# qianlim/CAPE

Measured on NVIDIA H100. Metric: meshes/sec fwd+bwd CAPE-affineconv nz64, higher is better.
Workload: dtype f32

## Files before the change

cape_b200/csrc/ellconv_dw_tc.cu:

```cuda
#include "common.cuh"
#include "ellconv_params.cuh"
#include "tc_common.cuh"

namespace cape {

namespace {

using namespace tc;

constexpr int DW_THREADS = 256;
constexpr int DW_KCH = 32;
constexpr int DW_A_TILE = 128 * 128;

struct DwTcParams {
  int rows_out, ncols, F, src_rows, src_stride;
  long long total_rows, rows_per_split;
  const float* src;
  OpView op;
  const float* g;
  float* out;
  long long out_rs;
  int nsplit, accumulate;
};

template <int BN>
struct DwCfg {
  static constexpr int G_TILE = BN * 128;
  static constexpr int STAGE = 2 * DW_A_TILE + 2 * G_TILE;
  static constexpr int SMEM_BYTES = 1024 + 2 * STAGE;
};

template <int BN>
__global__ void __launch_bounds__(DW_THREADS, BN <= 64 ? 2 : 1) dw_wg_kernel(const __grid_constant__ DwTcParams p) {
  using Cfg = DwCfg<BN>;
  constexpr int NA = BN / 2;
  constexpr int GQ = BN / 32;
  extern __shared__ uint8_t smem_raw[];
  char* smem = reinterpret_cast<char*>((reinterpret_cast<uintptr_t>(smem_raw) + 1023) & ~(uintptr_t)1023);

  const int tid = threadIdx.x, warp = tid >> 5, lane = tid & 31, wgi = tid >> 7, wt = tid & 127;
  const int ftile = blockIdx.x * 128;
  const int col0 = blockIdx.z * BN;
  const long long rbeg = (long long)blockIdx.y * p.rows_per_split;
  const long long rend = min(p.total_rows, rbeg + p.rows_per_split);
  const long long nchunks = (rend - rbeg + DW_KCH - 1) / DW_KCH;

  float4 ra[4], rg[GQ];
  auto load_chunk = [&](long long kc) {
    const long long R = rbeg + kc * DW_KCH + lane;
    const bool live = R < rend;
    const long long Q = live ? R : rbeg;
    const int n = (int)(Q / p.rows_out), r = (int)(Q % p.rows_out);
    const float* base = p.src + (size_t)n * p.src_rows * p.src_stride;
#pragma unroll
    for (int i = 0; i < 4; ++i) {
      const int f = ftile + 4 * (warp + 8 * i);
      float4 v = make_float4(0.f, 0.f, 0.f, 0.f);
      if (live && f < p.F) {
        if (p.op.idx == nullptr) v = ldg4(base + (size_t)r * p.src_stride + f);
        else ell_gather4(p.op, r, base + f, (size_t)p.src_stride, v);
      }
      ra[i] = v;
    }
#pragma unroll
    for (int i = 0; i < GQ; ++i) {
      const int c = col0 + 4 * (warp + 8 * i);
      rg[i] = make_float4(0.f, 0.f, 0.f, 0.f);
      if (live && c < p.ncols) rg[i] = ldg4(p.g + (size_t)R * p.ncols + c);
    }
  };
  auto store_chunk = [&](int stage) {
    char* a_hi = smem + (size_t)stage * Cfg::STAGE;
    char* a_lo = a_hi + DW_A_TILE;
    char* g_hi = a_lo + DW_A_TILE;
    char* g_lo = g_hi + Cfg::G_TILE;
#pragma unroll
    for (int i = 0; i < 4; ++i) {
      const int m = 4 * (warp + 8 * i);
      split_store1(ra[i].x, a_hi, a_lo, sw_off(m, lane));
      split_store1(ra[i].y, a_hi, a_lo, sw_off(m + 1, lane));
      split_store1(ra[i].z, a_hi, a_lo, sw_off(m + 2, lane));
      split_store1(ra[i].w, a_hi, a_lo, sw_off(m + 3, lane));
    }
#pragma unroll
    for (int i = 0; i < GQ; ++i) {
      const int m = 4 * (warp + 8 * i);
      split_store1(rg[i].x, g_hi, g_lo, sw_off(m, lane));
      split_store1(rg[i].y, g_hi, g_lo, sw_off(m + 1, lane));
      split_store1(rg[i].z, g_hi, g_lo, sw_off(m + 2, lane));
      split_store1(rg[i].w, g_hi, g_lo, sw_off(m + 3, lane));
    }
  };

  float acc[NA];
#pragma unroll
  for (int i = 0; i < NA; ++i) acc[i] = 0.f;

  if (nchunks > 0) {
    load_chunk(0);
    store_chunk(0);
    fence_proxy_async();
    __syncthreads();
    for (long long kc = 0;; ++kc) {
      const int stage = (int)(kc & 1);
      const uint32_t base = smem_u32(smem + (size_t)stage * Cfg::STAGE);
      const uint32_t a_hi = base + (uint32_t)(wgi * 64 * 128), a_lo = a_hi + DW_A_TILE;
      const uint32_t g_hi = base + 2 * DW_A_TILE, g_lo = g_hi + Cfg::G_TILE;
      wgmma_fence();
      fence_acc(acc);
      mma3_chunk<BN>(acc, a_hi, a_lo, g_hi, g_lo, 1);
      wgmma_commit();
      const bool more = kc + 1 < nchunks;
      if (more) {
        load_chunk(kc + 1);
        store_chunk(stage ^ 1);
      }
      wgmma_wait_all();
      fence_acc(acc);
      if (!more) break;
      fence_proxy_async();
      __syncthreads();
    }
  }

  float* out = p.out + (p.nsplit > 1 ? (size_t)blockIdx.y * p.F * p.out_rs : 0);
  const bool vec2 = (p.out_rs % 2 == 0) && ((reinterpret_cast<uintptr_t>(out) & 7u) == 0);
#pragma unroll
  for (int i = 0; i < NA; i += 2) {
    const int f = ftile + wgi * 64 + frag_row(wt, i);
    const int c = col0 + frag_col(wt, i);
    if (f >= p.F || c >= p.ncols) continue;
    float* o = out + (size_t)f * p.out_rs + c;
    if (p.nsplit == 1 && p.accumulate) {
      o[0] += acc[i];
      o[1] += acc[i + 1];
    } else if (vec2) {
      *reinterpret_cast<float2*>(o) = make_float2(acc[i], acc[i + 1]);
    } else {
      o[0] = acc[i];
      o[1] = acc[i + 1];
    }
  }
}

template <int BN>
int launch_dw(const DwTcParams& p, int ftiles, cudaStream_t st) {
  using Cfg = DwCfg<BN>;
  static bool configured = false;
  if (!configured) {
    CAPE_CHECK_CUDA(cudaFuncSetAttribute(dw_wg_kernel<BN>, cudaFuncAttributeMaxDynamicSharedMemorySize, Cfg::SMEM_BYTES));
    configured = true;
  }
  dim3 grid(ftiles, p.nsplit, (p.ncols + BN - 1) / BN);
  dw_wg_kernel<BN><<<grid, DW_THREADS, Cfg::SMEM_BYTES, st>>>(p);
  CAPE_CHECK_CUDA(cudaGetLastError());
  count_launches(1);
  return 1;
}

}

int launch_ellconv_dw_tc(const cape_topology* t, const cape_dw_args* a, const OpView& op, int* nsplit_out,
                         cudaStream_t st) {
  if (!tensor_cores_enabled()) return 0;
  if (a->ncols % 32 != 0 || a->ncols < 32 || a->ncols > 512) return 0;
  if (a->F % 4 != 0 || a->F < 32 || a->src_stride % 4 != 0 || !aligned16(a->src) || !aligned16(a->g)) return 0;
  DwTcParams p{};
  p.rows_out = a->rows_out; p.ncols = a->ncols; p.F = a->F; p.src_rows = a->src_rows; p.src_stride = a->src_stride;
  p.total_rows = (long long)a->N * a->rows_out;
  if (p.total_rows < 4096 || p.total_rows >= (1LL << 31)) return 0;
  p.src = a->src; p.op = op; p.g = a->g;
  const int BN = a->ncols <= 32 ? 32 : (a->ncols <= 64 ? 64 : (a->ncols <= 128 ? 128 : 256));
  const int ftiles = (a->F + 127) / 128, ctiles = (a->ncols + BN - 1) / BN;
  long long nsplit = (2LL * t->sm_count + ftiles * ctiles - 1) / (ftiles * ctiles);
  const long long max_by_rows = (p.total_rows + 511) / 512;
  if (nsplit > max_by_rows) nsplit = max_by_rows;
  const long long per = (long long)a->F * a->ncols * (long long)sizeof(float);
  if (nsplit > 1 && nsplit * per > t->workspace_bytes) nsplit = t->workspace_bytes / per;
  if (nsplit < 1) nsplit = 1;
  long long rps = (p.total_rows + nsplit - 1) / nsplit;
  rps = (rps + DW_KCH - 1) / DW_KCH * DW_KCH;
  nsplit = (p.total_rows + rps - 1) / rps;
  p.rows_per_split = rps; p.nsplit = (int)nsplit; p.accumulate = a->accumulate;
  if (nsplit == 1) { p.out = a->dw; p.out_rs = a->dw_stride; }
  else { p.out = (float*)t->workspace; p.out_rs = a->ncols; }
  *nsplit_out = (int)nsplit;
  if (BN == 32) return launch_dw<32>(p, ftiles, st);
  if (BN == 64) return launch_dw<64>(p, ftiles, st);
  if (BN == 128) return launch_dw<128>(p, ftiles, st);
  return launch_dw<256>(p, ftiles, st);
}

}
```

cape_b200/csrc/tc_common.cuh:

```cuda
#pragma once
#include <stdint.h>
#include "../../include/cape_b200.h"
#include "wgmma_tf32.cuh"

namespace cape {
namespace tc {

__device__ __forceinline__ uint32_t smem_u32(const void* p) { return (uint32_t)__cvta_generic_to_shared(p); }

__device__ __forceinline__ uint64_t make_desc(uint32_t smem_addr) {
  return (uint64_t)((smem_addr >> 4) & 0x3fffu) | (1ull << 16) | ((uint64_t)(1024 >> 4) << 32) | (1ull << 62);
}

__device__ __forceinline__ uint32_t sw_off(int m, int k) {
  return (uint32_t)(m * 128 + ((((k >> 2) ^ (m & 7)) << 4) | ((k & 3) << 2)));
}

__device__ __forceinline__ void fence_proxy_async() { asm volatile("fence.proxy.async.shared::cta;" ::: "memory"); }
__device__ __forceinline__ void wgmma_fence() { asm volatile("wgmma.fence.sync.aligned;" ::: "memory"); }
__device__ __forceinline__ void wgmma_commit() { asm volatile("wgmma.commit_group.sync.aligned;" ::: "memory"); }
__device__ __forceinline__ void wgmma_wait_all() { asm volatile("wgmma.wait_group.sync.aligned 0;" ::: "memory"); }

__device__ __forceinline__ void mbar_init(uint64_t* bar, int count) {
  asm volatile("mbarrier.init.shared::cta.b64 [%0], %1;" ::"r"(smem_u32(bar)), "r"(count) : "memory");
}
__device__ __forceinline__ void mbar_arrive(uint64_t* bar) {
  asm volatile("mbarrier.arrive.shared::cta.b64 _, [%0];" ::"r"(smem_u32(bar)) : "memory");
}
__device__ __forceinline__ void mbar_wait(uint64_t* bar, uint32_t parity) {
  uint32_t done;
  do {
    asm volatile("{\n\t.reg .pred p;\n\tmbarrier.try_wait.parity.shared::cta.b64 p, [%1], %2;\n\tselp.u32 %0, 1, 0, p;\n\t}"
                 : "=r"(done) : "r"(smem_u32(bar)), "r"(parity) : "memory");
  } while (!done);
}
__device__ __forceinline__ void named_bar_sync(int id, int nthreads) {
  asm volatile("bar.sync %0, %1;" ::"r"(id), "r"(nthreads) : "memory");
}
template <int N>
__device__ __forceinline__ void setmaxnreg_dec() { asm volatile("setmaxnreg.dec.sync.aligned.u32 %0;" ::"n"(N)); }
template <int N>
__device__ __forceinline__ void setmaxnreg_inc() { asm volatile("setmaxnreg.inc.sync.aligned.u32 %0;" ::"n"(N)); }

template <int N>
__device__ __forceinline__ void fence_acc(float (&d)[N]) {
#pragma unroll
  for (int i = 0; i < N; ++i) asm volatile("" : "+f"(d[i])::"memory");
}

__device__ __forceinline__ float tf32_hi(float x) { return __uint_as_float(__float_as_uint(x) & 0xffffe000u); }

__device__ __forceinline__ void split_store4(float4 v, char* hi_tile, char* lo_tile, uint32_t off) {
  float4 h, l;
  h.x = tf32_hi(v.x); l.x = v.x - h.x;
  h.y = tf32_hi(v.y); l.y = v.y - h.y;
  h.z = tf32_hi(v.z); l.z = v.z - h.z;
  h.w = tf32_hi(v.w); l.w = v.w - h.w;
  *reinterpret_cast<float4*>(hi_tile + off) = h;
  *reinterpret_cast<float4*>(lo_tile + off) = l;
}
__device__ __forceinline__ void split_store1(float v, char* hi_tile, char* lo_tile, uint32_t off) {
  const float h = tf32_hi(v);
  *reinterpret_cast<float*>(hi_tile + off) = h;
  *reinterpret_cast<float*>(lo_tile + off) = v - h;
}

template <int N>
__device__ __forceinline__ void mma3_chunk(float (&d)[N / 2], uint32_t a_hi, uint32_t a_lo, uint32_t b_hi,
                                           uint32_t b_lo, int scale_first) {
#pragma unroll
  for (int ks = 0; ks < 4; ++ks) {
    const uint32_t adv = 32u * ks;
    wg::mma_tf32<N>(d, make_desc(a_hi + adv), make_desc(b_hi + adv), ks == 0 ? scale_first : 1);
    wg::mma_tf32<N>(d, make_desc(a_lo + adv), make_desc(b_hi + adv), 1);
    wg::mma_tf32<N>(d, make_desc(a_hi + adv), make_desc(b_lo + adv), 1);
  }
}

__device__ __forceinline__ int frag_row(int t, int i) { return 16 * (t >> 5) + ((t & 31) >> 2) + 8 * ((i >> 1) & 1); }
__device__ __forceinline__ int frag_col(int t, int i) { return 8 * (i >> 2) + 2 * (t & 3) + (i & 1); }

}
}
```

cape_b200/network.py:

```python
import math
import os

import numpy as np
import torch

from . import _lib
from . import engine as E
from . import topology as topo
from .engine import (ACT_LEAKY, ACT_NONE, EPI_AFFINE, EPI_DUALMASK, EPI_LINEAR, EPI_SLOPE, ConvSite, Topology,
                     act_bwd, axpy, cheb_call, cheb_dw, colsum, gemm)
from .params import init_params, is_d_param, is_g_param, param_specs


ADAM_BETA1, ADAM_BETA2, ADAM_EPS = float(np.float32(0.9)), float(np.float32(0.999)), 1e-8


def _pad4(n):
    return (n + 3) // 4 * 4


class ParamStore:

    def __init__(self, specs, names, device):
        self.names = list(names)
        self.shapes = {n: tuple(specs[n]) for n in self.names}
        self.offsets = {}
        off = 0
        for n in self.names:
            self.offsets[n] = off
            off += _pad4(int(np.prod(self.shapes[n])))
        self.size = max(off, 4)
        self.flat = torch.zeros(self.size, device=device)
        self.grad = torch.zeros(self.size, device=device)
        self.mom = torch.zeros(self.size, device=device)
        self.lo = torch.zeros(self.size, device=device)
        self.var = None

    def add_adam_slot(self):
        if self.var is None:
            self.var = torch.zeros(self.size, device=self.flat.device)

    def lo_of(self, t):
        off = (t.data_ptr() - self.flat.data_ptr()) // 4
        if t.data_ptr() < self.flat.data_ptr() or off + t.numel() > self.size or not t.is_contiguous():
            return None
        return self.lo[off: off + t.numel()].view(t.shape)

    def _view(self, buf, n):
        k = int(np.prod(self.shapes[n]))
        return buf[self.offsets[n]: self.offsets[n] + k]

    def w(self, n):
        return self._view(self.flat, n)

    def g(self, n):
        return self._view(self.grad, n)

    def load(self, values):
        for n in self.names:
            self.w(n).copy_(torch.as_tensor(np.asarray(values[n], np.float32).reshape(-1)))

    def export(self, buf=None):
        buf = self.flat if buf is None else buf
        return {n: self._view(buf, n).detach().cpu().numpy().reshape(self.shapes[n]).copy() for n in self.names}


class Arena:

    def __init__(self):
        self.reqs = []
        self.buf = None

    def request(self, *shape):
        self.reqs.append(shape)
        return len(self.reqs) - 1

    def build(self, device):
        offs, off = [], 0
        for s in self.reqs:
            offs.append(off)
            off += _pad4(int(np.prod(s)))
        self.buf = torch.zeros(max(off, 4), device=device)
        self.views = [self.buf[o: o + int(np.prod(s))].view(*s) for o, s in zip(offs, self.reqs)]

    def get(self, i):
        return self.views[i]

    def zero(self):
        self.buf.zero_()


def choose_dw_mode(F, Fout, K, rows_in, rows_out, need_dx, stash=True):
    dense_ok = F % 4 == 0 and F >= 32 and Fout % 32 == 0 and Fout <= 512
    if not (dense_ok and stash):
        return "gather"
    if rows_out < rows_in:
        return "aside"
    if need_dx and (rows_in < rows_out or (K * Fout <= 512 and F >= Fout)):
        return "gside"
    return "aside"


def choose_forms(F, C, Fout, K, rows_in, rows_out, affine, need_dx, dw_mode, plain, name="", env=None):
    env = os.environ if env is None else env
    thin = F <= 4 or Fout <= 4
    split_ok = not thin and not plain and F % 16 == 0 and Fout % 16 == 0 and F >= 32 and Fout >= 32
    fwd_mode, dx_mode = "fused", "fused"
    basis_ok = C == 0 and not affine and dw_mode == "aside"
    if split_ok:
        if basis_ok and K >= 3 and rows_out < rows_in:
            fwd_mode = "basis"
        elif (C > 0 or affine) and rows_in < rows_out:
            fwd_mode = "contract"
        if (need_dx and not affine and dw_mode == "aside" and K * F <= 512
                and (Fout > F or (rows_out < rows_in and Fout == F and F >= 128))):
            dx_mode = "contract"
        if need_dx and dw_mode == "gside" and rows_in < rows_out and Fout >= 128:
            dx_mode = "basis"
    fm, dm = env.get("CAPE_FWD_MODE", ""), env.get("CAPE_DX_MODE", "")
    for item in filter(None, env.get("CAPE_MODES", "").split(",")):
        key, val = item.split("=")
        if key == name + ":fwd":
            fm = val
        elif key == name + ":dx":
            dm = val
    if fm and (fm == "fused" or (split_ok and (fm != "basis" or basis_ok))):
        fwd_mode = fm
    if dm and need_dx and (dm == "fused" or (split_ok and (dm != "basis" or dw_mode == "gside")
                                             and (dm != "contract" or (dw_mode != "gside" and not affine)))):
        dx_mode = dm
    return fwd_mode, dx_mode


class ChebLayer:

    def __init__(self, net, site, F, C, Fout, W, gW, bias=None, gbias=None, act=ACT_NONE, Wa=None, gWa=None,
                 bias_per_row=False, need_dx=True, maxN=1, n_cs_slots=1, name=""):
        self.net, self.tp, self.site, self.name = net, net.tp, site, name
        if (bias is not None or act != ACT_NONE) and not site.pool_is_selection:
            raise NotImplementedError("%s: the down-sampling matrix is not a pure row selection, so pooling cannot be "
                                      "folded in front of the bias/activation (lib/models.py:164-168 applies them "
                                      "before the pool)" % name)
        self.F, self.C, self.Fout, self.K = F, C, Fout, site.K
        K = self.K
        self.W3, self.gW3 = W.view(F + C, K, Fout), gW.view(F + C, K, Fout)
        self.W, self.bias, self.gbias, self.act = W, bias, gbias, act
        self.bias_per_row = bias_per_row
        self.affine = Wa is not None
        if self.affine:
            self.Wa, self.Wa2, self.gWa2 = Wa, Wa.view(F + C, Fout), gWa.view(F + C, Fout)
        self.need_dx = need_dx
        dev = W.device
        A = 1 if self.affine else 0
        self.Wt, self.Wt_lo = torch.empty(K + A, Fout, F, device=dev), torch.empty(K + A, Fout, F, device=dev)
        self.W3_lo = net.lo_of(W).view(F + C, K, Fout)
        net.wprep.add(W, F, K, Fout, wt=self.Wt[:K], wt_lo=self.Wt_lo[:K])
        if self.affine:
            self.Wa2_lo = net.lo_of(Wa).view(F + C, Fout)
            net.wprep.add(Wa, F, 1, Fout, wt=self.Wt[K:], wt_lo=self.Wt_lo[K:])
        self.dw_mode = choose_dw_mode(F, Fout, K, site.rows_in, site.rows_out, need_dx,
                                      os.environ.get("CAPE_DW_STASH", "1") != "0")
        self.stash_a, self.stash_g, self.stash_ga = [None] * K, [None] * K, None
        if self.dw_mode == "aside":
            nz = [k for k in range(K) if site.ops[k] != -1]
            self.stash_all = torch.empty(max(len(nz), 1), maxN, site.rows_out, F, device=dev)
            self.stash_a = [None] * K
            for j, k in enumerate(nz):
                self.stash_a[k] = self.stash_all[j]
        elif self.dw_mode == "gside":
            self.g_merged = K > 1 and K * Fout <= 512
            if self.g_merged:
                self.Hg = torch.empty(maxN, site.rows_in, K * Fout, device=dev)
                self.stash_g = [self.Hg[:, :, k * Fout:(k + 1) * Fout] for k in range(K)]
            else:
                self.stash_g = [None if site.opsT[k] == -1 else torch.empty(maxN, site.rows_in, Fout, device=dev)
                                for k in range(K)]
            if self.affine and site.opsT[0] != -1:
                self.stash_ga = torch.empty(maxN, site.rows_in, Fout, device=dev)
        self.fwd_mode, self.dx_mode = choose_forms(F, C, Fout, K, site.rows_in, site.rows_out, self.affine, need_dx,
                                                   self.dw_mode, all(o == -1 for o in site.ops), name)
        if self.dx_mode == "contract":
            self.Wk, self.Wk_lo = torch.empty(K, F, Fout, device=dev), torch.empty(K, F, Fout, device=dev)
            net.wprep.add(W, F, K, Fout, wk=self.Wk, wk_lo=self.Wk_lo)
            net.scratch_req(maxN * site.rows_out * K * F)
        if self.fwd_mode == "contract":
            net.scratch_req(maxN * site.rows_in * (K + A) * Fout)
        self.cs_ops = []
        if bias is not None and not bias_per_row:
            self.cs_ops.append(-1)
        self.cs_cond0 = len(self.cs_ops)
        if C:
            self.cs_ops += list(site.ops)
        self.cs_id = [net.arena.request(maxN, max(len(self.cs_ops), 1), Fout) for _ in range(n_cs_slots)]
        self.csa_id = net.arena.request(maxN, 1, Fout) if (self.affine and C) else None

    def alg_bytes(self, N, what):
        s, Fin, Fo, K = self.site, self.F + self.C, self.Fout, self.K
        wbytes = 4 * Fin * K * Fo + (12 * s.nnz if K > 1 else 0)
        conv = 4 * N * s.M * (Fin + Fo) + wbytes
        if self.affine:
            conv += 4 * N * s.M * (Fin + Fo) + 4 * Fin * Fo
            wbytes += 4 * Fin * Fo
        res = 0
        if s.ref_unpool:
            res += 4 * N * Fin * (s.ref_rows_in + s.M)
        if s.ref_pool:
            res += 4 * N * Fo * (s.M + s.ref_rows_out)
        if what in ("fwd", "dx"):
            return conv + res
        return 4 * N * s.M * Fin * (2 if self.affine else 1) + wbytes

    def _split(self):
        return E.tensor_cores_enabled(self.tp)

    def fwd(self, x, ycat, out, out2=None):
        N = x.shape[0]
        s, F, C, K, Fout = self.site, self.F, self.C, self.K, self.Fout
        assert x.shape[1] == s.rows_in and x.shape[2] >= F and out.shape[1] == s.rows_out
        sx = x.shape[2]
        tag = (self.name + ":fwd", self.alg_bytes(N, "fwd"))
        sub = lambda what: (self.name + ":fwd/" + what, 0)
        if self.fwd_mode == "contract" and self._split():
            A = 1 if self.affine else 0
            ncz = (K + A) * Fout
            Z = self.net.scratch[: N * s.rows_in * ncz].view(N, s.rows_in, ncz)
            cheb_call(self.tp, N, s.rows_in, ncz,
                      [dict(src=x, op=-1, F=F, src_rows=s.rows_in, src_stride=sx, w=None, w_stride=0,
                            wT=self.Wt.view(ncz, F), wT_stride=F, wT_lo=self.Wt_lo.view(ncz, F))],
                      Z, plain_only=True, tag=sub("project"))
            terms = [dict(src=Z[:, :, k * Fout:], op=s.ops[k], src_rows=s.rows_in, src_stride=ncz, acc=0,
                          wc=self.W3[F:, k, :] if C else None, wc_stride=K * Fout) for k in range(K)]
            if self.affine:
                terms.append(dict(src=Z[:, :, K * Fout:], op=s.ops[0], src_rows=s.rows_in, src_stride=ncz, acc=1,
                                  wc=self.Wa2[F:] if C else None, wc_stride=Fout))
            E.apply_call(self.tp, N, s.rows_out, Fout, terms, out, out2=out2, cond=ycat if C else None,
                         epilogue=EPI_AFFINE if self.affine else EPI_LINEAR, act=self.act, bias=self.bias,
                         bias_per_row=self.bias_per_row, tag=tag)
            return
        basis = self.fwd_mode == "basis" and self._split()
        if basis:
            nz = [k for k in range(K) if s.ops[k] != -1]
            if N == self.stash_all.shape[1]:
                E.apply_call(self.tp, N, s.rows_out, F, [dict(src=x, op=s.ops[k], src_rows=s.rows_in, src_stride=sx) for k in nz],
                             self.stash_all, term_stride=self.stash_all.stride(0), tag=sub("basis"))
            else:
                for k in nz:
                    E.apply_call(self.tp, N, s.rows_out, F, [dict(src=x, op=s.ops[k], src_rows=s.rows_in, src_stride=sx)],
                                 self.stash_a[k][:N], tag=sub("basis%d" % k))
        terms = []
        for k in range(K):
            t = dict(src=x, op=s.ops[k], F=F, src_rows=s.rows_in, src_stride=sx, w=self.W3[:, k, :],
                     w_stride=K * Fout, wT=self.Wt[k], wT_stride=F, wT_lo=self.Wt_lo[k])
            if C:
                t["wc"] = self.W3[F:, k, :]
            if basis and s.ops[k] != -1:
                t.update(src=self.stash_a[k][:N], op=-1, src_rows=s.rows_out, src_stride=F)
            elif self.stash_a[k] is not None:
                t["stash"], t["stash_stride"] = self.stash_a[k][:N], F
            if self.affine and k == 0:
                t["w2"], t["w2_stride"] = self.Wa2, Fout
                t["w2T"], t["w2T_stride"], t["w2T_lo"] = self.Wt[K], F, self.Wt_lo[K]
                if C:
                    t["wc2"] = self.Wa2[F:]
            terms.append(t)
        cheb_call(self.tp, N, s.rows_out, Fout, terms, out, out2=out2, cond=ycat if C else None,
                  epilogue=EPI_AFFINE if self.affine else EPI_LINEAR, act=self.act, bias=self.bias,
                  bias_per_row=self.bias_per_row, tag=tag)

    def bwd(self, x, ycat, g, g_aff=None, dx=None, dx2=None, dx_epi=EPI_LINEAR, dx_aux=None, dx_alpha=E.LEAKY_ALPHA,
            dycat=None, want_dw=True, cs_slot=0):
        tp, s, F, C, K, Fout = self.tp, self.site, self.F, self.C, self.K, self.Fout
        N = g.shape[0]
        sx = x.shape[2]
        mode = self.dw_mode if (want_dw and (self.dw_mode != "gside" or dx is not None)) else "gather"
        if want_dw and mode == "aside":
            nl = K + (1 if self.affine else 0)
            tg = (self.name + ":dW", self.alg_bytes(N, "dW") / nl)

            def dw_aside(tp):
                for k in range(K):
                    B = self.stash_a[k]
                    if B is None:
                        cheb_dw(tp, N, s.rows_out, Fout, x, -1, F, s.rows_in, sx, g, self.gW3[:, k, :], K * Fout, tag=tg)
                    else:
                        cheb_dw(tp, N, s.rows_out, Fout, B[:N], -1, F, s.rows_out, F, g, self.gW3[:, k, :], K * Fout,
                                tag=tg)
                if self.affine:
                    B = self.stash_a[0]
                    if B is None:
                        cheb_dw(tp, N, s.rows_out, Fout, x, -1, F, s.rows_in, sx, g_aff, self.gWa2, Fout, tag=tg)
                    else:
                        cheb_dw(tp, N, s.rows_out, Fout, B[:N], -1, F, s.rows_out, F, g_aff, self.gWa2, Fout, tag=tg)
            self.net.run_dw(dw_aside)
        elif (want_dw and mode == "gather" and Fout <= 4 and not self.affine and F in (32, 64, 128, 256) and sx == F
              and K <= 4):
            cheb_dw(tp, N, s.rows_in, F, g, list(s.opsT), Fout, s.rows_out, Fout, x, self.gW3, 1,
                    tag=(self.name + ":dW", self.alg_bytes(N, "dW")), dw_term_stride=Fout, dw_col_stride=K * Fout)
        elif want_dw and mode == "gather":
            nl = (1 if F <= 4 else K) + (1 if self.affine else 0)
            tg = (self.name + ":dW", self.alg_bytes(N, "dW") / nl)
            if F <= 4:
                cheb_dw(tp, N, s.rows_out, Fout, x, list(s.ops), F, s.rows_in, sx, g, self.gW3, K * Fout, tag=tg,
# ... 435 lines not shown
    def lo_of(self, t):
        r = self.PG.lo_of(t)
        return r if r is not None else self.PD.lo_of(t)

    def prep_weights(self):
        E.tf32_lo(self.tp, self.PG.flat, self.PG.lo)
        E.tf32_lo(self.tp, self.PD.flat, self.PD.lo)
        self.wprep.run()

    def scratch_req(self, nfloats):
        self._scratch_need = max(getattr(self, "_scratch_need", 4), int(nfloats))

    def set_inputs(self, x_g, cond_g, cond2_g, eps, x_d=None, cond_d=None, cond2_d=None, non_blocking=True):
        N = self.N
        self.in_x.copy_(x_g, non_blocking=non_blocking)
        self.in_cond[N:].copy_(cond_g, non_blocking=non_blocking)
        self.in_cond2[N:].copy_(cond2_g, non_blocking=non_blocking)
        self.in_eps.copy_(eps, non_blocking=non_blocking)
        if x_d is not None:
            self.xcat[:N].copy_(x_d, non_blocking=non_blocking)
            self.in_cond[:N].copy_(cond_d, non_blocking=non_blocking)
            self.in_cond2[:N].copy_(cond2_d, non_blocking=non_blocking)

    def prefetch_inputs(self, x_g, cond_g, cond2_g, eps, x_d=None, cond_d=None, cond2_d=None):
        if not hasattr(self, "_stage"):
            bufs = (self.in_x, self.in_cond[self.N:], self.in_cond2[self.N:], self.in_eps, self.xcat[:self.N],
                    self.in_cond[:self.N], self.in_cond2[:self.N])
            self._stage = [[torch.empty_like(b) for b in bufs] for _ in range(2)]
            self._stage_ev = [torch.cuda.Event(), torch.cuda.Event()]
            self._stage_free = [torch.cuda.Event(), torch.cuda.Event()]
            self._copy_stream = torch.cuda.Stream(device=self.device)
            self._stage_slot = 0
            for e in self._stage_free:
                e.record()
        slot = self._stage_slot
        self._copy_stream.wait_event(self._stage_free[slot])
        srcs = (x_g, cond_g, cond2_g, eps) if x_d is None else (x_g, cond_g, cond2_g, eps, x_d, cond_d, cond2_d)
        self._stage_n = len(srcs)
        with torch.cuda.stream(self._copy_stream):
            for dst, src in zip(self._stage[slot], srcs):
                dst.copy_(src, non_blocking=True)
            self._stage_ev[slot].record(self._copy_stream)

    def commit_inputs(self):
        slot = self._stage_slot
        cur = torch.cuda.current_stream()
        cur.wait_event(self._stage_ev[slot])
        self.set_inputs(*self._stage[slot][: self._stage_n])
        self._stage_free[slot].record(cur)
        self._stage_slot = 1 - slot

    def cond_fwd(self, lo, hi):
        nzc = self.cfg["nz_cond"]
        self.c_pose1.fwd(self.in_cond[lo:hi], self.cp_h[lo:hi])
        self.c_pose2.fwd(self.cp_h[lo:hi], self.ycat[lo:hi, :nzc])
        if self.c_clo2 is None:
            self.c_clo1.fwd(self.in_cond2[lo:hi], self.ycat[lo:hi, nzc:])
        else:
            self.c_clo1.fwd(self.in_cond2[lo:hi], self.cc_h[lo:hi])
            self.c_clo2.fwd(self.cc_h[lo:hi], self.ycat[lo:hi, nzc:])

    def encoder_fwd(self):
        x = self.in_x
        for l, a in zip(self.enc, self.enc_act):
            l.fwd(x, None, a)
            x = a
        self.enc_1x1.fwd(x, None, self.enc_red)
        flat = self.enc_red.view(self.N, self.flat)
        self.fc_mean.fwd(flat, self.z_mean)
        self.fc_var.fwd(flat, self.z_logvar)

    def sample_fwd(self):
        N, nz = self.N, self.nz
        _lib.check(self.tp.lib.cape_vae_sample_fwd(E._ptr(self.z_mean), E._ptr(self.z_logvar), E._ptr(self.in_eps),
                                                   E._ptr(self.z_total), nz + self.Cc, N, nz, E._stream()))
        self.z_total[:, nz:].copy_(self.ycat_g)

    def decoder_fwd(self, z_total=None, ycat=None, out=None):
        z_total = self.z_total if z_total is None else z_total
        ycat = self.ycat_g if ycat is None else ycat
        out = self.x_hat if out is None else out
        self.dec_fc1.fwd(z_total, self.dec_fc)
        self.dec_1x1.fwd(self.dec_fc.view(self.N, self.p[-1], self.red), None, self.dec_h0)
        x = self.dec_h0
        if self.affine:
            for l, a, rg in zip(self.dec, self.dec_act, self.dec_rg):
                l.fwd(x, ycat, a, out2=rg)
                x = a
        else:
            for b, a in zip(self.dec, self.dec_act):
                b.fwd(x, ycat, a)
                x = a
        self.dec_out.fwd(x, ycat, out)

    def disc_fwd(self, lo, hi):
        x = self.xcat[lo:hi]
        yc = self.ycat[lo:hi]
        for l, a in zip(self.disc, self.disc_act):
            l.fwd(x, yc, a[lo:hi])
            x = a[lo:hi]
        self.disc_pred.fwd(x, None, self.logits[lo:hi])

    def disc_bwd(self, lo, hi, dlogits, want_dw, dx=None, dycat=None, cs_slot=0):
        n = len(self.disc)
        acts = [a[lo:hi] for a in self.disc_act]
        gs = [gb[: hi - lo] for gb in self.g_disc]
        yc = self.ycat[lo:hi]
        self.disc_pred.bwd(acts[-1], None, dlogits, dx=gs[-1], dx_epi=EPI_SLOPE, dx_aux=acts[-1], want_dw=want_dw,
                           cs_slot=cs_slot)
        for i in range(n - 1, 0, -1):
            self.disc[i].bwd(acts[i - 1], None, gs[i], dx=gs[i - 1], dx_epi=EPI_SLOPE, dx_aux=acts[i - 1],
                             want_dw=want_dw, cs_slot=cs_slot)
        self.disc[0].bwd(self.xcat[lo:hi], yc, gs[0], dx=dx, dycat=dycat, want_dw=want_dw, cs_slot=cs_slot)

    def decoder_bwd(self):
        N, nl = self.N, len(self.dec)
        yc = self.ycat_g
        last = self.dec_act[-1]
        if not self.affine:
            self.dec_out.bwd(last, yc, self.d_xhat, dx=self.g_dec[-1], dycat=self.d_ycat)
            for i in range(nl - 1, -1, -1):
                x = self.dec_act[i - 1] if i > 0 else self.dec_h0
                self.dec[i].bwd(x, yc, self.g_dec[i], self.g_dec[i - 1] if i > 0 else self.g_dec_h0, self.d_ycat)
        else:
            self.dec_out.bwd(last, yc, self.d_xhat, dx=self.g_dec[-1], dx2=self.g_dec_m[-1], dx_epi=EPI_DUALMASK,
                             dx_aux=self.dec_rg[-1], dycat=self.d_ycat)
        for i in range(nl - 1 if self.affine else -1, -1, -1):
            x = self.dec_act[i - 1] if i > 0 else self.dec_h0
            if i > 0:
                self.dec[i].bwd(x, yc, self.g_dec_m[i], g_aff=self.g_dec[i], dx=self.g_dec[i - 1],
                                dx2=self.g_dec_m[i - 1], dx_epi=EPI_DUALMASK, dx_aux=self.dec_rg[i - 1],
                                dycat=self.d_ycat)
            else:
                self.dec[i].bwd(x, yc, self.g_dec_m[i], g_aff=self.g_dec[i], dx=self.g_dec_h0, dycat=self.d_ycat)
        fcv = self.dec_fc.view(N, self.p[-1], self.red)
        self.dec_1x1.bwd(fcv, None, self.g_dec_h0, dx=self.g_dec_fc.view(N, self.p[-1], self.red))
        self.dec_fc1.bwd(self.z_total, self.dec_fc, self.g_dec_fc, gtmp=self.g_dec_fc_t)
        W = self.dec_fc1.W
        gemm(self.tp, self.g_dec_fc_t, W[:self.nz].t(), self.g_z)
        gemm(self.tp, self.g_dec_fc_t, W[self.nz:].t(), self.d_ycat, beta=1.0)

    def encoder_bwd(self):
        N, nz = self.N, self.nz
        c = self.cfg
        _lib.check(self.tp.lib.cape_vae_sample_bwd(E._ptr(self.g_z), nz, E._ptr(self.z_mean),
                                                   E._ptr(self.z_logvar), E._ptr(self.in_eps), E._ptr(self.g_mean),
                                                   E._ptr(self.g_logvar), N, nz, float(c["lambda_latent"]),
                                                   E._stream()))
        flat = self.enc_red.view(N, self.flat)
        gflat = self.g_enc_red.view(N, self.flat)
        self.fc_mean.bwd(flat, self.z_mean, self.g_mean, dx=gflat)
        self.fc_var.bwd(flat, self.z_logvar, self.g_logvar, dx=gflat, dx_beta=1.0)
        self._fc_reg(("generator/encoder/fc_mean", "generator/encoder/fc_var"))
        self._reduce_bucket("enc_fc")
        self.enc_1x1.bwd(self.enc_act[-1], None, self.g_enc_red, dx=self.g_enc[-1], dx_epi=EPI_SLOPE,
                         dx_aux=self.enc_act[-1])
        for i in range(len(self.enc) - 1, 0, -1):
            self.enc[i].bwd(self.enc_act[i - 1], None, self.g_enc[i], dx=self.g_enc[i - 1], dx_epi=EPI_SLOPE,
                            dx_aux=self.enc_act[i - 1])
        self.enc[0].bwd(self.in_x, None, self.g_enc[0])

    def cond_bwd(self):
        N = self.N
        nzc = self.cfg["nz_cond"]
        dy = self.d_ycat[:, :nzc]
        dy2 = self.d_ycat[:, nzc:]
        self.c_pose2.bwd(self.cp_h[N:], None, dy, dx=self.g_cp_h)
        self.c_pose1.bwd(self.in_cond[N:], self.cp_h[N:], self.g_cp_h, gtmp=self.g_cp_t)
        if self.c_clo2 is None:
            self.c_clo1.bwd(self.in_cond2[N:], None, dy2)
        else:
            self.c_clo2.bwd(self.cc_h[N:], None, dy2, dx=self.g_cc_h)
            self.c_clo1.bwd(self.in_cond2[N:], self.cc_h[N:], self.g_cc_h, gtmp=self.g_cc_t)

    def forward_generator(self):
        N = self.N
        self.cond_fwd(N, 2 * N)
        self.encoder_fwd()
        self.sample_fwd()
        self.decoder_fwd()
        return self.x_hat

    def lr_now(self, step):
        c = self.cfg
        lr_g, lr_d = c["lr"], c["lr"] * c["lr_scaler"]
        ds = int(c["decay_steps"])
        if c["lr_warmup"]:
            warm = int(c["decay_steps"] * 8)
            if step < warm:
                return lr_g * step / warm, lr_d * step / warm
            k = math.floor((step - warm) / ds)
        else:
            k = math.floor(step / ds)
        return lr_g * c["decay_rate"] ** k, lr_d * c["decay_rate"] ** k

    def enqueue_fwd_bwd(self):
        N, c, tp = self.N, self.cfg, self.tp
        lam_gan = float(c["lambda_gan"])
        self.arena.zero()
        self.losses.zero_()
        self.d_ycat.zero_()
        if not self.affine:
            self.PG.grad.zero_()
        self.cond_fwd(0, 2 * N)
        self.encoder_fwd()
        self.sample_fwd()
        self.decoder_fwd()
        self.disc_fwd(0, 2 * N)
        nlog = N * self.p_d[-1]
        L = self.losses
        lib = tp.lib
        st = E._stream
        _lib.check(lib.cape_bce_logits(E._ptr(self.logits[N:]), nlog, 0.9, lam_gan, E._ptr(self.d_logits_g),
                                       E._ptr(L[3:]), st()))
        _lib.check(lib.cape_bce_logits(E._ptr(self.logits[:N]), nlog, 0.9, lam_gan, E._ptr(self.d_logits[:N]),
                                       E._ptr(L[4:]), st()))
        _lib.check(lib.cape_bce_logits(E._ptr(self.logits[N:]), nlog, 0.1, lam_gan, E._ptr(self.d_logits[N:]),
                                       E._ptr(L[5:]), st()))
        if not self.ref_compat:
            self.disc_bwd(0, 2 * N, self.d_logits, want_dw=True)
        self.join_dw()
        self.disc_bwd(N, 2 * N, self.d_logits_g, want_dw=False, dx=self.d_xhat, dycat=self.d_ycat, cs_slot=1)
        _lib.check(lib.cape_recon_losses(tp.h, self.nbr_op, E._ptr(self.x_hat), E._ptr(self.in_x), N, self.p[0],
                                         float(c["lambda_recon"]), float(c["lambda_edge"]), self.n_edges,
                                         E._ptr(self.z_mean), E._ptr(self.z_logvar), self.nz, E._ptr(self.d_xhat),
                                         E._ptr(L), st()))
        self.decoder_bwd()
        self._fc_reg(("generator/decoder/fc1",))
        if not self.side_glue:
            self.small.flush()
        self._reduce_bucket("dec")
        self.encoder_bwd()
        self.join_dw()
        self.small.flush()
        self.cond_bwd()
        if self.ref_compat:
            self.PD.grad.copy_(self.PD.flat)
        if not c["optim_condnet"]:
            for n in self.PG.names:
                if not n.startswith("generator"):
                    self.PG.g(n).zero_()
        self._reduce_bucket("rest")
        if self.dp is not None:
            torch.cuda.current_stream().wait_stream(self.dp["stream"])

    def _fc_reg(self, names):
        r2 = float(self.cfg["regularization"]) ** 2
        if r2 > 0:
            for n in names:
                axpy(self.tp, self._g(n + "/dense/kernel"), self._w(n + "/dense/kernel"), r2)

    def set_data_parallel(self, world):
        if world <= 1:
            self.dp = None
            return
        self.side_glue = False
        P = self.PG
        names = P.names
        fc0 = P.offsets["generator/encoder/fc_mean/dense/kernel"]
        dec0 = P.offsets[next(n for n in names if n.startswith("generator/decoder"))]
        assert fc0 < dec0 and all(P.offsets[n] >= dec0 for n in names if n.startswith("generator/decoder"))
        self.dp = dict(world=world, stream=torch.cuda.Stream(device=self.device),
                       buckets={"dec": [P.grad[dec0:]] + ([] if self.ref_compat else [self.PD.grad]),
                                "enc_fc": [P.grad[fc0:dec0]], "rest": [P.grad[:fc0]]})

    def _reduce_bucket(self, which):
        if self.dp is None:
            return
        import torch.distributed as dist
        comm = self.dp["stream"]
        comm.wait_stream(torch.cuda.current_stream())
        if self._dw_pending:
            comm.wait_stream(self.dw_stream)
        with torch.cuda.stream(comm):
            for b in self.dp["buckets"][which]:
                dist.all_reduce(b, op=dist.ReduceOp.AVG)

    def enqueue_update(self):
        lib = self.tp.lib
        self.sumsq.zero_()
        for P, i in ((self.PG, 0), (self.PD, 1)):
            _lib.check(lib.cape_sumsq(E._ptr(P.grad), P.size, E._ptr(self.sumsq[i:]), E._stream()))
            if self.adam:
                _lib.check(lib.cape_adam_clip_update(E._ptr(P.flat), E._ptr(P.grad), E._ptr(P.mom), E._ptr(P.var), P.size,
                                                     E._ptr(self.sumsq[i:]), 5.0, E._ptr(self.lr[i:]), ADAM_BETA1,
                                                     ADAM_BETA2, ADAM_EPS, E._stream()))
            else:
                _lib.check(lib.cape_sgd_clip_update(E._ptr(P.flat), E._ptr(P.grad), E._ptr(P.mom), P.size,
                                                    E._ptr(self.sumsq[i:]), 5.0, E._ptr(self.lr[i:]),
                                                    float(self.cfg["momentum"]), E._stream()))
        self.prep_weights()

    def set_lr(self, step):
        lr_g, lr_d = self.lr_now(step)
        if self.adam:
            t = self.adam_t + 1
            corr = math.sqrt(1.0 - ADAM_BETA2 ** t) / (1.0 - ADAM_BETA1 ** t)
            lr_g, lr_d = lr_g * corr, lr_d * corr
        slot = self._lr_host[self._lr_slot]
        self._lr_slot = (self._lr_slot + 1) % self._lr_host.shape[0]
        slot[0], slot[1] = lr_g, lr_d
        self.lr.copy_(slot, non_blocking=True)

    def capture_graphs(self):
        self.graph_fb, self.graph_up = torch.cuda.CUDAGraph(), torch.cuda.CUDAGraph()
        torch.cuda.synchronize()
        with torch.cuda.graph(self.graph_fb):
            self.enqueue_fwd_bwd()
        with torch.cuda.graph(self.graph_up):
            self.enqueue_update()
        torch.cuda.synchronize()

    def capture_forward_graph(self):
        self.graph_fwd = torch.cuda.CUDAGraph()
        torch.cuda.synchronize()
        with torch.cuda.graph(self.graph_fwd):
            self.forward_generator()
        torch.cuda.synchronize()

    def train_step(self, step=None, update=True, allreduce=None, use_graph=False):
        step = self.step_count if step is None else step
        if update:
            self.set_lr(step)
        if use_graph:
            self.graph_fb.replay()
        else:
            self.enqueue_fwd_bwd()
        if allreduce is not None and self.dp is None:
            allreduce(self.PG.grad, self.PD.grad)
        if update:
            if use_graph:
                self.graph_up.replay()
            else:
                self.enqueue_update()
            self.step_count = step + 1
            self.adam_t += 1
        return self.losses

    def loss_dict(self):
        v = self.losses.detach().cpu().numpy()
        c = self.cfg
        out = dict(recon=float(v[0]), edge=float(v[1]), latent=float(v[2]), gan_g=float(v[3]),
                   gan_d=float(v[4] + v[5]))
        out["loss_g_noreg"] = (out["gan_g"] * c["lambda_gan"] + out["recon"] * c["lambda_recon"]
                               + out["edge"] * c["lambda_edge"] + out["latent"] * c["lambda_latent"])
        out["loss_d"] = out["gan_d"] * c["lambda_gan"]
        return out


def _adjacency(L):
    import scipy.sparse as sp
    A = sp.csr_matrix(L, copy=True)
    A.setdiag(0)
    A.eliminate_zeros()
    A.data[:] = 1.0
    return A
```

Baseline: 2054.

## Warp-specialize dW tensor-core kernel with mbarrier multi-stage producer/consumer ring

Reworks the weight-gradient TF32 wgmma kernel into a warp-specialized design. Dedicated producer warpgroups gather, split and store chunks into a multi-stage shared-memory ring synchronized by full/empty mbarriers, while two consumer warpgroups issue wgmma with one group in flight. Registers are rebalanced between the roles with setmaxnreg, and the grid is flattened to 1D. The intent is to overlap global gathers with tensor-core work, which the old double-buffered, __syncthreads-coupled loop serialized. In exchange it uses more shared memory and allows only one block per SM. It also disables Python GC during CUDA graph capture, a robustness change.

New measurement: 2131, median of 6. +3.8%, better.

```diff
diff --git a/cape_b200/csrc/ellconv_dw_tc.cu b/cape_b200/csrc/ellconv_dw_tc.cu
--- a/cape_b200/csrc/ellconv_dw_tc.cu
+++ b/cape_b200/csrc/ellconv_dw_tc.cu
@@ -8,9 +8,10 @@
 
 using namespace tc;
 
-constexpr int DW_THREADS = 256;
 constexpr int DW_KCH = 32;
 constexpr int DW_A_TILE = 128 * 128;
+constexpr int DW_BAR_BYTES = 256;
+constexpr int DW_SMEM_MAX = 227 * 1024;
 
 struct DwTcParams {
   int rows_out, ncols, F, src_rows, src_stride;
@@ -21,113 +22,141 @@
   float* out;
   long long out_rs;
   int nsplit, accumulate;
+  int ftiles, ctiles;
 };
 
 template <int BN>
 struct DwCfg {
   static constexpr int G_TILE = BN * 128;
   static constexpr int STAGE = 2 * DW_A_TILE + 2 * G_TILE;
-  static constexpr int SMEM_BYTES = 1024 + 2 * STAGE;
+  static constexpr int STAGES = (DW_SMEM_MAX - 1024 - DW_BAR_BYTES) / STAGE;
+  static constexpr int RING = STAGES * STAGE;
+  static constexpr int SMEM_BYTES = 1024 + RING + DW_BAR_BYTES;
+  static constexpr int PRODUCERS = BN <= 128 ? 2 : 1;
+  static constexpr int THREADS = 128 * (PRODUCERS + 2);
+  static constexpr int PRODUCER_REGS = BN <= 128 ? 120 : 152;
+  static constexpr int CONSUMER_REGS = BN <= 128 ? 136 : 176;
+  static_assert(PRODUCERS * PRODUCER_REGS + 2 * CONSUMER_REGS <= (PRODUCERS + 2) * (65536 / THREADS / 8 * 8),
+                "register split exceeds the launch budget");
+  static_assert(STAGES >= 2, "the ring needs at least two stages");
+  static_assert(2 * STAGES * 8 <= DW_BAR_BYTES, "mbarrier area too small");
 };
 
 template <int BN>
-__global__ void __launch_bounds__(DW_THREADS, BN <= 64 ? 2 : 1) dw_wg_kernel(const __grid_constant__ DwTcParams p) {
+__global__ void __launch_bounds__(DwCfg<BN>::THREADS, 1) dw_wg_kernel(const __grid_constant__ DwTcParams p) {
   using Cfg = DwCfg<BN>;
+  constexpr int S = Cfg::STAGES;
   constexpr int NA = BN / 2;
-  constexpr int GQ = BN / 32;
+  constexpr int GQ = BN / 16;
   extern __shared__ uint8_t smem_raw[];
   char* smem = reinterpret_cast<char*>((reinterpret_cast<uintptr_t>(smem_raw) + 1023) & ~(uintptr_t)1023);
-
-  const int tid = threadIdx.x, warp = tid >> 5, lane = tid & 31, wgi = tid >> 7, wt = tid & 127;
-  const int ftile = blockIdx.x * 128;
-  const int col0 = blockIdx.z * BN;
-  const long long rbeg = (long long)blockIdx.y * p.rows_per_split;
+  uint64_t* full = reinterpret_cast<uint64_t*>(smem + Cfg::RING);
+  uint64_t* empty = full + S;
+
+  const int tid = threadIdx.x, wgi = tid >> 7, lane = tid & 31;
+  const int ct = (int)(blockIdx.x % (unsigned)p.ctiles);
+  const int ft = (int)(blockIdx.x / (unsigned)p.ctiles % (unsigned)p.ftiles);
+  const int split = (int)(blockIdx.x / (unsigned)(p.ctiles * p.ftiles));
+  const int ftile = ft * 128;
+  const int col0 = ct * BN;
+  const long long rbeg = (long long)split * p.rows_per_split;
   const long long rend = min(p.total_rows, rbeg + p.rows_per_split);
   const long long nchunks = (rend - rbeg + DW_KCH - 1) / DW_KCH;
 
-  float4 ra[4], rg[GQ];
-  auto load_chunk = [&](long long kc) {
-    const long long R = rbeg + kc * DW_KCH + lane;
-    const bool live = R < rend;
-    const long long Q = live ? R : rbeg;
-    const int n = (int)(Q / p.rows_out), r = (int)(Q % p.rows_out);
-    const float* base = p.src + (size_t)n * p.src_rows * p.src_stride;
-#pragma unroll
-    for (int i = 0; i < 4; ++i) {
-      const int f = ftile + 4 * (warp + 8 * i);
-      float4 v = make_float4(0.f, 0.f, 0.f, 0.f);
-      if (live && f < p.F) {
-        if (p.op.idx == nullptr) v = ldg4(base + (size_t)r * p.src_stride + f);
-        else ell_gather4(p.op, r, base + f, (size_t)p.src_stride, v);
-      }
-      ra[i] = v;
+  if (tid == 0) {
+    for (int s = 0; s < S; ++s) {
+      mbar_init(&full[s], 128);
+      mbar_init(&empty[s], 8);
     }
-#pragma unroll
-    for (int i = 0; i < GQ; ++i) {
-      const int c = col0 + 4 * (warp + 8 * i);
-      rg[i] = make_float4(0.f, 0.f, 0.f, 0.f);
-      if (live && c < p.ncols) rg[i] = ldg4(p.g + (size_t)R * p.ncols + c);
+  }
+  __syncthreads();
+
+  if (wgi < Cfg::PRODUCERS) {
+    setmaxnreg_dec<Cfg::PRODUCER_REGS>();
+    const int w4 = (tid >> 5) & 3;
+    const int kr = 16 * (w4 & 1) + (lane >> 1), g0 = 2 * (w4 >> 1) + (lane & 1);
+    uint32_t off[4];
+#pragma unroll
+    for (int e = 0; e < 4; ++e) off[e] = sw_off(4 * g0 + e, kr);
+    for (long long kc = wgi; kc < nchunks; kc += Cfg::PRODUCERS) {
+      const int R = (int)(rbeg + kc * DW_KCH) + kr;
+      const bool live = R < rend;
+      const int Q = live ? R : (int)rbeg;
+      const int n = Q / p.rows_out, r = Q % p.rows_out;
+      const float* base = p.src + (size_t)n * p.src_rows * p.src_stride;
+      float4 ra[8], rg[GQ];
+#pragma unroll
+      for (int i = 0; i < GQ; ++i) {
+        const int c = col0 + 4 * (g0 + 4 * i);
+        rg[i] = make_float4(0.f, 0.f, 0.f, 0.f);
+        if (live && c < p.ncols) rg[i] = ldg4(p.g + (size_t)R * p.ncols + c);
+      }
+#pragma unroll
+      for (int i = 0; i < 8; ++i) {
+        const int f = ftile + 4 * (g0 + 4 * i);
+        float4 v = make_float4(0.f, 0.f, 0.f, 0.f);
+        if (live && f < p.F) {
+          if (p.op.idx == nullptr) v = ldg4(base + (size_t)r * p.src_stride + f);
+          else ell_gather4(p.op, r, base + f, (size_t)p.src_stride, v);
+        }
+        ra[i] = v;
+      }
+      const int stage = (int)(kc % S);
+      mbar_wait(&empty[stage], (uint32_t)((kc / S) & 1) ^ 1);
+      char* a_hi = smem + (size_t)stage * Cfg::STAGE;
+      char* a_lo = a_hi + DW_A_TILE;
+      char* g_hi = a_lo + DW_A_TILE;
+      char* g_lo = g_hi + Cfg::G_TILE;
+#pragma unroll
+      for (int i = 0; i < 8; ++i) {
+        char* hi = a_hi + 2048 * i;
+        char* lo = a_lo + 2048 * i;
+        split_store1(ra[i].x, hi, lo, off[0]);
+        split_store1(ra[i].y, hi, lo, off[1]);
+        split_store1(ra[i].z, hi, lo, off[2]);
+        split_store1(ra[i].w, hi, lo, off[3]);
+      }
+#pragma unroll
+      for (int i = 0; i < GQ; ++i) {
+        char* hi = g_hi + 2048 * i;
+        char* lo = g_lo + 2048 * i;
+        split_store1(rg[i].x, hi, lo, off[0]);
+        split_store1(rg[i].y, hi, lo, off[1]);
+        split_store1(rg[i].z, hi, lo, off[2]);
+        split_store1(rg[i].w, hi, lo, off[3]);
+      }
+      fence_proxy_async();
+      mbar_arrive(&full[stage]);
     }
-  };
-  auto store_chunk = [&](int stage) {
-    char* a_hi = smem + (size_t)stage * Cfg::STAGE;
-    char* a_lo = a_hi + DW_A_TILE;
-    char* g_hi = a_lo + DW_A_TILE;
-    char* g_lo = g_hi + Cfg::G_TILE;
-#pragma unroll
-    for (int i = 0; i < 4; ++i) {
-      const int m = 4 * (warp + 8 * i);
-      split_store1(ra[i].x, a_hi, a_lo, sw_off(m, lane));
-      split_store1(ra[i].y, a_hi, a_lo, sw_off(m + 1, lane));
-      split_store1(ra[i].z, a_hi, a_lo, sw_off(m + 2, lane));
-      split_store1(ra[i].w, a_hi, a_lo, sw_off(m + 3, lane));
-    }
-#pragma unroll
-    for (int i = 0; i < GQ; ++i) {
-      const int m = 4 * (warp + 8 * i);
-      split_store1(rg[i].x, g_hi, g_lo, sw_off(m, lane));
-      split_store1(rg[i].y, g_hi, g_lo, sw_off(m + 1, lane));
-      split_store1(rg[i].z, g_hi, g_lo, sw_off(m + 2, lane));
-      split_store1(rg[i].w, g_hi, g_lo, sw_off(m + 3, lane));
-    }
-  };
-
+    return;
+  }
+
+  setmaxnreg_inc<Cfg::CONSUMER_REGS>();
+  const int cw = wgi - Cfg::PRODUCERS, wt = tid & 127;
   float acc[NA];
 #pragma unroll
   for (int i = 0; i < NA; ++i) acc[i] = 0.f;
-
-  if (nchunks > 0) {
-    load_chunk(0);
-    store_chunk(0);
-    fence_proxy_async();
-    __syncthreads();
-    for (long long kc = 0;; ++kc) {
-      const int stage = (int)(kc & 1);
-      const uint32_t base = smem_u32(smem + (size_t)stage * Cfg::STAGE);
-      const uint32_t a_hi = base + (uint32_t)(wgi * 64 * 128), a_lo = a_hi + DW_A_TILE;
-      const uint32_t g_hi = base + 2 * DW_A_TILE, g_lo = g_hi + Cfg::G_TILE;
-      wgmma_fence();
-      fence_acc(acc);
-      mma3_chunk<BN>(acc, a_hi, a_lo, g_hi, g_lo, 1);
-      wgmma_commit();
-      const bool more = kc + 1 < nchunks;
-      if (more) {
-        load_chunk(kc + 1);
-        store_chunk(stage ^ 1);
-      }
-      wgmma_wait_all();
-      fence_acc(acc);
-      if (!more) break;
-      fence_proxy_async();
-      __syncthreads();
-    }
-  }
-
-  float* out = p.out + (p.nsplit > 1 ? (size_t)blockIdx.y * p.F * p.out_rs : 0);
+  fence_acc(acc);
+  for (long long kc = 0; kc < nchunks; ++kc) {
+    const int stage = (int)(kc % S);
+    mbar_wait(&full[stage], (uint32_t)((kc / S) & 1));
+    const uint32_t base = smem_u32(smem + (size_t)stage * Cfg::STAGE);
+    const uint32_t a_hi = base + (uint32_t)(cw * 64 * 128), a_lo = a_hi + DW_A_TILE;
+    const uint32_t g_hi = base + 2 * DW_A_TILE, g_lo = g_hi + Cfg::G_TILE;
+    wgmma_fence();
+    mma3_chunk<BN>(acc, a_hi, a_lo, g_hi, g_lo, 1);
+    wgmma_commit();
+    wgmma_wait<1>();
+    if (kc > 0 && lane == 0) mbar_arrive(&empty[(int)((kc - 1) % S)]);
+  }
+  wgmma_wait<0>();
+  fence_acc(acc);
+
+  float* out = p.out + (p.nsplit > 1 ? (size_t)split * p.F * p.out_rs : 0);
   const bool vec2 = (p.out_rs % 2 == 0) && ((reinterpret_cast<uintptr_t>(out) & 7u) == 0);
 #pragma unroll
   for (int i = 0; i < NA; i += 2) {
-    const int f = ftile + wgi * 64 + frag_row(wt, i);
+    const int f = ftile + cw * 64 + frag_row(wt, i);
     const int c = col0 + frag_col(wt, i);
     if (f >= p.F || c >= p.ncols) continue;
     float* o = out + (size_t)f * p.out_rs + c;
@@ -144,15 +173,19 @@
 }
 
 template <int BN>
-int launch_dw(const DwTcParams& p, int ftiles, cudaStream_t st) {
+int launch_dw(const DwTcParams& p, cudaStream_t st) {
   using Cfg = DwCfg<BN>;
   static bool configured = false;
   if (!configured) {
     CAPE_CHECK_CUDA(cudaFuncSetAttribute(dw_wg_kernel<BN>, cudaFuncAttributeMaxDynamicSharedMemorySize, Cfg::SMEM_BYTES));
     configured = true;
   }
-  dim3 grid(ftiles, p.nsplit, (p.ncols + BN - 1) / BN);
-  dw_wg_kernel<BN><<<grid, DW_THREADS, Cfg::SMEM_BYTES, st>>>(p);
+  const long long nblocks = (long long)p.ftiles * p.ctiles * p.nsplit;
+  if (nblocks >= (1LL << 31)) {
+    set_error("dw_wg_kernel: too many tiles");
+    return -1;
+  }
+  dw_wg_kernel<BN><<<(unsigned)nblocks, Cfg::THREADS, Cfg::SMEM_BYTES, st>>>(p);
   CAPE_CHECK_CUDA(cudaGetLastError());
   count_launches(1);
   return 1;
@@ -171,8 +204,9 @@
   if (p.total_rows < 4096 || p.total_rows >= (1LL << 31)) return 0;
   p.src = a->src; p.op = op; p.g = a->g;
   const int BN = a->ncols <= 32 ? 32 : (a->ncols <= 64 ? 64 : (a->ncols <= 128 ? 128 : 256));
-  const int ftiles = (a->F + 127) / 128, ctiles = (a->ncols + BN - 1) / BN;
-  long long nsplit = (2LL * t->sm_count + ftiles * ctiles - 1) / (ftiles * ctiles);
+  p.ftiles = (a->F + 127) / 128;
+  p.ctiles = (a->ncols + BN - 1) / BN;
+  long long nsplit = (2LL * t->sm_count + p.ftiles * p.ctiles - 1) / (p.ftiles * p.ctiles);
   const long long max_by_rows = (p.total_rows + 511) / 512;
   if (nsplit > max_by_rows) nsplit = max_by_rows;
   const long long per = (long long)a->F * a->ncols * (long long)sizeof(float);
@@ -185,10 +219,10 @@
   if (nsplit == 1) { p.out = a->dw; p.out_rs = a->dw_stride; }
   else { p.out = (float*)t->workspace; p.out_rs = a->ncols; }
   *nsplit_out = (int)nsplit;
-  if (BN == 32) return launch_dw<32>(p, ftiles, st);
-  if (BN == 64) return launch_dw<64>(p, ftiles, st);
-  if (BN == 128) return launch_dw<128>(p, ftiles, st);
-  return launch_dw<256>(p, ftiles, st);
-}
-
-}
+  if (BN == 32) return launch_dw<32>(p, st);
+  if (BN == 64) return launch_dw<64>(p, st);
+  if (BN == 128) return launch_dw<128>(p, st);
+  return launch_dw<256>(p, st);
+}
+
+}
diff --git a/cape_b200/csrc/tc_common.cuh b/cape_b200/csrc/tc_common.cuh
--- a/cape_b200/csrc/tc_common.cuh
+++ b/cape_b200/csrc/tc_common.cuh
@@ -20,6 +20,8 @@
 __device__ __forceinline__ void wgmma_fence() { asm volatile("wgmma.fence.sync.aligned;" ::: "memory"); }
 __device__ __forceinline__ void wgmma_commit() { asm volatile("wgmma.commit_group.sync.aligned;" ::: "memory"); }
 __device__ __forceinline__ void wgmma_wait_all() { asm volatile("wgmma.wait_group.sync.aligned 0;" ::: "memory"); }
+template <int N>
+__device__ __forceinline__ void wgmma_wait() { asm volatile("wgmma.wait_group.sync.aligned %0;" ::"n"(N) : "memory"); }
 
 __device__ __forceinline__ void mbar_init(uint64_t* bar, int count) {
   asm volatile("mbarrier.init.shared::cta.b64 [%0], %1;" ::"r"(smem_u32(bar)), "r"(count) : "memory");
diff --git a/cape_b200/network.py b/cape_b200/network.py
--- a/cape_b200/network.py
+++ b/cape_b200/network.py
@@ -1,3 +1,5 @@
+import contextlib
+import gc
 import math
 import os
 
@@ -1039,20 +1041,34 @@
         slot[0], slot[1] = lr_g, lr_d
         self.lr.copy_(slot, non_blocking=True)
 
+    @staticmethod
+    @contextlib.contextmanager
+    def _no_collector():
+        gc.collect()
+        was_enabled = gc.isenabled()
+        gc.disable()
+        try:
+            yield
+        finally:
+            if was_enabled:
+                gc.enable()
+
     def capture_graphs(self):
         self.graph_fb, self.graph_up = torch.cuda.CUDAGraph(), torch.cuda.CUDAGraph()
         torch.cuda.synchronize()
-        with torch.cuda.graph(self.graph_fb):
-            self.enqueue_fwd_bwd()
-        with torch.cuda.graph(self.graph_up):
-            self.enqueue_update()
+        with self._no_collector():
+            with torch.cuda.graph(self.graph_fb):
+                self.enqueue_fwd_bwd()
+            with torch.cuda.graph(self.graph_up):
+                self.enqueue_update()
         torch.cuda.synchronize()
 
     def capture_forward_graph(self):
         self.graph_fwd = torch.cuda.CUDAGraph()
         torch.cuda.synchronize()
-        with torch.cuda.graph(self.graph_fwd):
-            self.forward_generator()
+        with self._no_collector():
+            with torch.cuda.graph(self.graph_fwd):
+                self.forward_generator()
         torch.cuda.synchronize()
 
     def train_step(self, step=None, update=True, allreduce=None, use_graph=False):
```
